# David-OConnor/molchanica

Hardware: AMD Instinct MI355X
Metric: MD atom-updates/sec (and steps/sec), 1M-atom solvated box (higher is better)
Workload: dtype f32

## Files before the change

molchanica_amd/csrc/mdx_nonbonded_impl.h:

```cpp
#pragma once
#include "mdx_internal.h"
#include "mdx_bonded_dev.h"
#include "mdx_pair_dev.h"
#include <algorithm>
#include <cfloat>
#include <cstdlib>
#include <type_traits>

constexpr int NB_WAVES = MDX_NB_WAVES;
#ifdef NB_DRAIN_TRACE
extern uint4* g_mdx_drain; extern size_t g_mdx_drain_cap; extern uint32_t g_mdx_drain_n; extern int g_mdx_drain_on;
#endif
#ifndef NB_ASM_PAIR
#define NB_ASM_PAIR 0
#endif
#ifndef NB_HALF_FLUSH
#define NB_HALF_FLUSH 0
#endif

template <bool BIAS, bool R2OUT>
__device__ __forceinline__ void pair_eval_asm(float xi, float yi, float zi, float qi, float sgi, float epi, const float4 pj,
                                              const float2 lj, float rc2, float bias, float& fx, float& fy, float& fz,
                                              float& g0, float& g1, float& g2, float& r2_out) {
    float dx, dy, dz, r2, t1, t2, t3, t4;
    if (BIAS) {
        asm volatile(
            "v_sub_f32 %[dy], %[yi], %[yj]\n\t"
            "v_sub_f32 %[dx], %[xi], %[xj]\n\t"
            "v_fma_f32 %[r2], %[dy], %[dy], %[bias]\n\t"
            "v_sub_f32 %[dz], %[zi], %[zj]\n\t"
            "v_fmac_f32 %[r2], %[dx], %[dx]\n\t"
            "v_fmac_f32 %[r2], %[dz], %[dz]\n\t"
            : [dx] "=&v"(dx), [dy] "=&v"(dy), [dz] "=&v"(dz), [r2] "=&v"(r2)
            : [xi] "v"(xi), [yi] "v"(yi), [zi] "v"(zi), [xj] "v"(pj.x), [yj] "v"(pj.y), [zj] "v"(pj.z), [bias] "v"(bias));
    } else {
        asm volatile(
            "v_sub_f32 %[dy], %[yi], %[yj]\n\t"
            "v_sub_f32 %[dx], %[xi], %[xj]\n\t"
            "v_mul_f32 %[r2], %[dy], %[dy]\n\t"
            "v_sub_f32 %[dz], %[zi], %[zj]\n\t"
            "v_fmac_f32 %[r2], %[dx], %[dx]\n\t"
            "v_fmac_f32 %[r2], %[dz], %[dz]\n\t"
            : [dx] "=&v"(dx), [dy] "=&v"(dy), [dz] "=&v"(dz), [r2] "=&v"(r2)
            : [xi] "v"(xi), [yi] "v"(yi), [zi] "v"(zi), [xj] "v"(pj.x), [yj] "v"(pj.y), [zj] "v"(pj.z));
    }
    if (R2OUT) r2_out = r2;
    asm volatile(
        "v_cmpx_gt_f32 vcc, %[rc2], %[r2]\n\t"
        "v_rsq_f32 %[r2], %[r2]\n\t"
        "v_add_f32 %[t1], %[sgi], %[ljx]\n\t"
        "v_mul_f32 %[t1], %[t1], %[t1]\n\t"
        "v_mul_f32 %[t2], %[epi], %[ljy]\n\t"
        "v_mul_f32 %[t3], %[r2], %[r2]\n\t"
        "v_mul_f32 %[t1], %[t1], %[t3]\n\t"
        "v_mul_f32 %[t4], %[t1], %[t1]\n\t"
        "v_mul_f32 %[t1], %[t1], %[t4]\n\t"
        "v_mul_f32 %[t2], %[t2], %[t1]\n\t"
        "v_fma_f32 %[t1], %[t1], 2.0, -1.0\n\t"
        "v_mul_f32 %[t1], %[t2], %[t1]\n\t"
        "v_mul_f32 %[t2], %[qi], %[qj]\n\t"
        "v_fmac_f32 %[t1], %[t2], %[r2]\n\t"
        "v_mul_f32 %[t1], %[t3], %[t1]\n\t"
        "v_fmac_f32 %[fx], %[dx], %[t1]\n\t"
        "v_fmac_f32 %[fy], %[dy], %[t1]\n\t"
        "v_fmac_f32 %[fz], %[dz], %[t1]\n\t"
        "v_fma_f32 %[g0], -%[dx], %[t1], %[g0]\n\t"
        "v_fma_f32 %[g1], -%[dy], %[t1], %[g1]\n\t"
        "v_fma_f32 %[g2], -%[dz], %[t1], %[g2]\n\t"
        "s_mov_b64 exec, -1\n\t"
        : [fx] "+v"(fx), [fy] "+v"(fy), [fz] "+v"(fz), [g0] "+v"(g0), [g1] "+v"(g1), [g2] "+v"(g2), [r2] "+v"(r2),
          [t1] "=&v"(t1), [t2] "=&v"(t2), [t3] "=&v"(t3), [t4] "=&v"(t4)
        : [rc2] "s"(rc2), [sgi] "v"(sgi), [epi] "v"(epi), [ljx] "v"(lj.x), [ljy] "v"(lj.y), [qi] "v"(qi), [qj] "v"(pj.w),
          [dx] "v"(dx), [dy] "v"(dy), [dz] "v"(dz)
        : "vcc");
}

template <bool ENERGY, int COUL, bool GEOM, bool SAMECUT, bool MASKED>
__device__ __forceinline__ void chunk_pairs(const float4* __restrict__ sx, const float2* __restrict__ sl,
                                            unsigned long long mask, float xi, float yi, float zi, float qi,
                                            float sgi, float epi, const NbParams& p, float& fx, float& fy,
                                            float& fz, double& elj, double& ecoul, double& evir) {
    float e1 = 0.f, e2 = 0.f, e3 = 0.f;
#pragma unroll 8
    for (int jj = 0; jj < 64; ++jj) {
        const bool allowed = MASKED ? (bool)((mask >> jj) & 1ull) : true;
        pair_eval<ENERGY, COUL, GEOM, SAMECUT, false>(xi, yi, zi, qi, sgi, epi, sx[jj], sl[jj], allowed, p, fx, fy, fz,
                                               e1, e2, nullptr, ENERGY ? &e3 : nullptr);
    }
    if (ENERGY) { elj += (double)e1; ecoul += (double)e2; evir += (double)e3; }
}

template <bool ENERGY, int COUL, bool GEOM, bool SAMECUT>
__global__ __launch_bounds__(NB_WAVES * 64) void nb_tile_kernel(NbArgs a) {
    if (a.gate && *a.gate > a.thr_bits) return;
    __shared__ float4 s_xyzq[NB_WAVES][64];
    __shared__ float2 s_lj[NB_WAVES][64];
    const int lane = threadIdx.x & 63, wave = threadIdx.x >> 6;
    const uint32_t nblocks = (a.T + NB_WAVES - 1) / NB_WAVES;
    const uint32_t per_xcd = (nblocks + 7) >> 3;
    const uint32_t blk = (blockIdx.x & 7u) * per_xcd + (blockIdx.x >> 3);
    if (blk >= nblocks) return;
    const uint32_t t = blk * NB_WAVES + wave;
    if (t >= a.T) return;

    const uint32_t islot = t * MDX_TILE + lane;
    const float4 pi = a.posq[islot];
    const float2 li = a.lj[islot];
    const ListCounts cnt = a.counts[t];
    const uint32_t e0 = a.entry_off[t];
    const uint32_t nmc = cnt.n_masked >> 3, nchunks = (cnt.n_masked + cnt.n_plain) >> 3;
    const uint32_t mbase = a.mchunk_off[t];
    float4* sx = s_xyzq[wave];
    float2* sl = s_lj[wave];

    float fx = 0.f, fy = 0.f, fz = 0.f;
    double elj = 0.0, ecoul = 0.0, evir = 0.0;

    float4 nj = make_float4(0.f, 0.f, 0.f, 0.f);
    float2 nl = make_float2(0.f, 0.f);
    uint32_t ncode = 13;
    if (nchunks) {
        const uint2 ent = a.entries[e0 + (lane >> 3)];
        const uint32_t js = ent.x * MDX_CLUSTER + (lane & 7);
        nj = a.posq[js]; nl = a.lj[js]; ncode = ent.y & 31u;
    }
    for (uint32_t c = 0; c < nchunks; ++c) {
        {
            const int kx = (int)(ncode % 3u) - 1, ky = (int)((ncode / 3u) % 3u) - 1, kz = (int)(ncode / 9u) - 1;
            nj.x += (float)kx * a.p.shift[0];
            nj.y += (float)ky * a.p.shift[1];
            nj.z += (float)kz * a.p.shift[2];
            sx[lane] = nj;
            sl[lane] = nl;
        }
        WAVE_LDS_SYNC();
        if (c + 1 < nchunks) {
            const uint2 ent = a.entries[e0 + (c + 1) * 8 + (lane >> 3)];
            const uint32_t js = ent.x * MDX_CLUSTER + (lane & 7);
            nj = a.posq[js]; nl = a.lj[js]; ncode = ent.y & 31u;
        }
        if (c < nmc) {
            const unsigned long long m = a.masks[(size_t)(mbase + c) * 64 + lane];
            chunk_pairs<ENERGY, COUL, GEOM, SAMECUT, true>(sx, sl, m, pi.x, pi.y, pi.z, pi.w, li.x, li.y, a.p,
                                                           fx, fy, fz, elj, ecoul, evir);
        } else {
            chunk_pairs<ENERGY, COUL, GEOM, SAMECUT, false>(sx, sl, ~0ull, pi.x, pi.y, pi.z, pi.w, li.x, li.y,
                                                            a.p, fx, fy, fz, elj, ecoul, evir);
        }
        WAVE_LDS_SYNC();
    }
    a.force[islot] = make_float4(fx, fy, fz, 0.f);
    if (ENERGY) {
        if (!(a.slot_flags[islot] & 2u)) { elj = 0.0; ecoul = 0.0; evir = 0.0; }
#pragma unroll
        for (int m = 32; m > 0; m >>= 1) {
            elj += __shfl_xor(elj, m);
            ecoul += __shfl_xor(ecoul, m);
            evir += __shfl_xor(evir, m);
        }
        if (lane == 0) {
            double* q = a.energy + EN_COUNT + 8 + MDX_ESTRIDE * (blk & (MDX_EPART - 1));
            atomicAdd(q, 0.5 * elj); atomicAdd(q + 1, 0.5 * ecoul); atomicAdd(q + 2, 0.5 * evir);
        }
    }
}


template <bool ENERGY, int COUL, bool GEOM, bool SAMECUT, int WPT, bool HALF, bool ALCH, int DUAL, int BW, bool STEP = false, bool UNI = false>
__device__ __forceinline__ void nb_cluster_body(const NbArgs& a, const bool owned_prune, float4 (*s_xyzq)[64], float4 (*s_lj)[64],
                                                float (*s_red)[3][64], float (*s_ownj)[64], float4 (*s_g)[64],
                                                unsigned long long (*s_mask)[64], const float4* __restrict__ etab = nullptr) {
    const int lane = threadIdx.x & 63, wave = __builtin_amdgcn_readfirstlane(threadIdx.x >> 6);
    constexpr int SPLIT = BW < WPT ? WPT / BW : 1;
    static_assert(!UNI || (!ENERGY && !GEOM && !ALCH && !STEP), "the constant-sigma^2 body: force-only, Lorentz-Berthelot, no alchemical window");
    static_assert(SPLIT == 1 || HALF, "a tile split over workgroups returns its i-forces through atomics");
    constexpr int TPB = SPLIT > 1 ? 1 : BW / WPT;
    const uint32_t ntiles = a.tile_order ? a.t_count : a.T;
    const uint32_t nblocks = SPLIT > 1 ? ntiles * SPLIT : (ntiles + TPB - 1) / TPB;
    const uint32_t per_xcd = (nblocks + 7) >> 3;
    constexpr bool TAIL = WPT == 1 && HALF && DUAL != 0 && !STEP && BW == 1;
    const bool tail_on = TAIL && a.tail_w > 1u;
    const uint32_t blk = (a.xcd_interleave || tail_on) ? blockIdx.x : (blockIdx.x & 7u) * per_xcd + (blockIdx.x >> 3);
    if (!tail_on && blk >= nblocks) return;
    const int tib = SPLIT > 1 ? 0 : wave / WPT;
// ... 68 lines not shown
                if (a.st_prune_out && !(pw <= a.st_path_thr)) *a.st_prune_out = 1u;
                if (any_viol) { *a.st_viol = 1u; if (a.st_disp_out) atomicMax(a.st_disp_out, __float_as_uint(1.0e20f)); }
            }
            if (WPT == 1 && a.b_role_off) {
                const uint32_t rb = a.b_role_off[s], re = a.b_role_off[s + 1];
                if (re > rb) {
                    float bx = 0.f, by = 0.f, bz = 0.f;
                    RoleEnergies en;
                    for (uint32_t k = rb; k < re; ++k) role_eval_step<false>(a.b_roles[k], a.b_prm, x, a.posq, a.st_fprev, a.b_p, bx, by, bz, en);
                    float* const fb_ = reinterpret_cast<float*>(a.force) + (size_t)s * 4;
                    unsafeAtomicAdd(fb_, bx); unsafeAtomicAdd(fb_ + 1, by); unsafeAtomicAdd(fb_ + 2, bz);
                }
            }
        }
        s_xyzq[wave][lane] = x;
        WAVE_LDS_SYNC();
#pragma unroll
        for (int ci = 0; ci < 8; ++ci) {
            const float4 pi = s_xyzq[wave][ci * MDX_CLUSTER + ii];
            const float2 li = a.lj[t * MDX_TILE + ci * MDX_CLUSTER + ii];
            xi[ci] = pi.x; yi[ci] = pi.y; zi[ci] = pi.z; qi[ci] = pi.w; sgi[ci] = li.x; epi[ci] = li.y;
            fx[ci] = 0.f; fy[ci] = 0.f; fz[ci] = 0.f;
        }
        WAVE_LDS_SYNC();
    } else {
#pragma unroll
    for (int ci = 0; ci < 8; ++ci) {
        const uint32_t s = t * MDX_TILE + ci * MDX_CLUSTER + ii;
        const float4 pi = a.posq[s];
        const float2 li = UNI ? make_float2(0.f, reinterpret_cast<const float*>(a.lj)[2 * s + 1]) : a.lj[s];
        xi[ci] = pi.x; yi[ci] = pi.y; zi[ci] = pi.z; qi[ci] = pi.w; sgi[ci] = li.x; epi[ci] = li.y;
        fx[ci] = 0.f; fy[ci] = 0.f; fz[ci] = 0.f;
    }
    }
    ListCounts cnt = a.counts[t_ok ? t : 0];
    if (!t_ok) { cnt.n_masked = 0; cnt.n_plain = 0; }
    const uint32_t e0 = a.entry_off[t_ok ? t : 0];
    const uint2* __restrict__ const entries = DUAL == 1 ? a.entries_in : a.entries;
    const uint32_t nmc = cnt.n_masked >> 3;
    const uint32_t nchunks = DUAL == 1 ? (t_ok ? a.inner_nch[t * 8 + part] : 0u) : (cnt.n_masked + cnt.n_plain) >> 3;
    const uint32_t mbase = a.mchunk_off[t_ok ? t : 0];
    float4* sx = s_xyzq[wave];
    float4* const sl = s_lj[wave];
    const float* __restrict__ const lj_eps = reinterpret_cast<const float*>(a.lj) + 1;
    double elj = 0.0, ecoul = 0.0, evir = 0.0, ecross = 0.0, edudl = 0.0;
    uint32_t own_bits = 0xFFu;
    if (ENERGY && !a.energy_all) {
        own_bits = 0;
#pragma unroll
        for (int ci = 0; ci < 8; ++ci)
            own_bits |= ((a.slot_flags[t * MDX_TILE + ci * MDX_CLUSTER + ii] >> 1) & 1u) << ci;
    }

    float4 nj = make_float4(0.f, 0.f, 0.f, 0.f), nf = nj;
    float2 nl = make_float2(0.f, 0.f);
    uint32_t ny = 13, njc = 0;
    float nown = 0.f;
    unsigned long long nmq = ~0ull;
    uint2 ent_n = make_uint2(0u, 13u);
    if ((uint32_t)part < nchunks) {
        const uint2 ent = entries[e0 + part * 8 + (lane >> 3)];
        if ((uint32_t)part < nmc) nmq = a.masks[(size_t)(mbase + part) * 64 + lane];
        if ((uint32_t)part + wv < nchunks) ent_n = entries[e0 + (part + wv) * 8 + (lane >> 3)];
        const uint32_t js = ent.x * MDX_CLUSTER + (lane & 7);
        nj = a.posq[js]; ny = ent.y; njc = ent.x;
        if (UNI) nl.y = lj_eps[2 * js]; else nl = a.lj[js];
        if (STEP) nf = a.st_fprev[js];
        if (ENERGY && HALF) nown = a.energy_all ? 1.0f : (float)((a.slot_flags[js] >> 1) & 1u);
    }
    float* const fbase = reinterpret_cast<float*>(a.force);
    const bool jsel_x = ii == 0 || ii == 7, jsel_y = ii == 1 || ii == 6;
    const uint32_t jlane_off = (uint32_t)(jj * 4 + ii) * 4u;
    float4* const sg = s_g[HALF ? wave : 0];
    constexpr bool prune = DUAL == 2;
    uint32_t kept = 0;
#ifdef NB_HALF_STATS
    uint32_t dbg_jh = 0, dbg_ih = 0, dbg_q = 0, dbg_pairs = 0;
#endif
    const uint32_t c_first = nmc + (TAIL ? (((uint32_t)part + wv - (nmc & (wv - 1u))) & (wv - 1u)) : ((uint32_t)part + WPT - nmc % WPT) % WPT);
    uint32_t wcur = 0;
    if (HALF && NB_HALF_FLUSH) __builtin_amdgcn_s_waitcnt(0x0F70);
    const float rc2_s = __builtin_bit_cast(float, __builtin_amdgcn_readfirstlane(__builtin_bit_cast(int, a.p.rc2_lj)));
    auto chunk_pass = [&](auto masked_tag, const uint32_t c_begin, const uint32_t c_end) __attribute__((always_inline)) {
    constexpr bool MASKED_CHUNK = decltype(masked_tag)::value;
    for (uint32_t c = c_begin; c < c_end; c += wv) {
        const uint32_t cur_y = ny, cur_jc = njc;
        constexpr bool masked = MASKED_CHUNK;
        if (masked) s_mask[wave][lane] = nmq;
        if (ENERGY && HALF) s_ownj[wave][lane] = nown;
        if (HALF && NB_HALF_FLUSH) {
            const bool live = ((ny >> 8) & 0xFFu) != 0u;
            sg[lane] = make_float4(0.f, 0.f, 0.f, __uint_as_float(live ? njc * MDX_CLUSTER + (uint32_t)ii : t * MDX_TILE + lane));
        }
        {
            const uint32_t code = ny & 31u;
            const int kx = (int)(code % 3u) - 1, ky = (int)((code / 3u) % 3u) - 1, kz = (int)(code / 9u) - 1;
            if (STEP) nj = step_pos(nj, nf);
            nj.x += (float)kx * a.p.shift[0];
            nj.y += (float)ky * a.p.shift[1];
            nj.z += (float)kz * a.p.shift[2];
            sx[lane] = nj;
            if (UNI) sl[lane].x = nl.y; else *reinterpret_cast<float2*>(&sl[lane]) = nl;
        }
        WAVE_LDS_SYNC();
        if (c + wv < nmc) nmq = a.masks[(size_t)(mbase + c + wv) * 64 + lane];
        if (c + wv < nchunks) {
            const uint32_t js = ent_n.x * MDX_CLUSTER + (lane & 7);
            nj = a.posq[js]; ny = ent_n.y; njc = ent_n.x;
            if (UNI) nl.y = lj_eps[2 * js]; else nl = a.lj[js];
            if (STEP) nf = a.st_fprev[js];
            if (ENERGY && HALF) nown = a.energy_all ? 1.0f : (float)((a.slot_flags[js] >> 1) & 1u);
            if (c + 2 * wv < nchunks) ent_n = entries[e0 + (c + 2 * wv) * 8 + (lane >> 3)];
        }
        float celj = 0.f, cecoul = 0.f, cevir = 0.f, cecross = 0.f, cedudl = 0.f;
        uint32_t newy = cur_y & 0xFFu;
#pragma unroll 1
        for (int e = 0; e < 8; ++e) {
            const float4 pj = sx[e * 8 + jj];
            const float2 lj = UNI ? make_float2(0.f, sl[e * 8 + jj].x) : *reinterpret_cast<const float2*>(&sl[e * 8 + jj]);
            const uint32_t im = (__builtin_amdgcn_readlane(cur_y, e * 8) >> 8) & 0xFFu;
            if (im == 0) continue;
            uint32_t newm = 0;
            const int x8 = MASKED_CHUNK ? (int)(~(uint32_t)reinterpret_cast<const uint8_t*>(&s_mask[wave][lane])[e]) : 0;
            float g[3] = {-0.f, -0.f, -0.f};
            float wj = 0.f;
            if (ENERGY && HALF) wj = 0.5f * s_ownj[wave][e * 8 + jj];
#pragma unroll
            for (int ci = 0; ci < 8; ++ci) {
                if (im & (1u << ci)) {
                    float e1 = 0.f, e2 = 0.f, e3 = 0.f, e4 = 0.f, e5 = 0.f;
                    const float bias = MASKED_CHUNK ? __int_as_float((x8 << (31 - ci)) >> 31) : 0.f;
                    float r2v = 0.f;
                    constexpr bool ASM_PAIR = NB_ASM_PAIR && !ENERGY && COUL == CM_SHIFTED && !GEOM && SAMECUT && HALF && !ALCH && !UNI;
                    if constexpr (ASM_PAIR)
                        pair_eval_asm<MASKED_CHUNK, prune>(xi[ci], yi[ci], zi[ci], qi[ci], sgi[ci], epi[ci], pj, lj, rc2_s, bias, fx[ci], fy[ci], fz[ci],
                                                           g[0], g[1], g[2], r2v);
                    else
                    pair_eval<ENERGY, COUL, GEOM, SAMECUT, true, HALF, ALCH, MASKED_CHUNK, UNI>(xi[ci], yi[ci], zi[ci], qi[ci], sgi[ci], epi[ci],
                                                                             pj, lj, true, a.p, fx[ci], fy[ci],
                                                                             fz[ci], e1, e2, g, ENERGY ? &e3 : nullptr,
                                                                             (ENERGY && ALCH) ? &e4 : nullptr, bias,
                                                                             prune ? &r2v : nullptr, (ENERGY && ALCH) ? &e5 : nullptr, etab);
                    if (prune) {
                        const unsigned long long bb = __ballot(r2v < a.rin2);
                        if (bb != 0ull) newm |= 1u << ci;
#ifdef NB_HALF_STATS
                        if (bb != 0ull) {
                            const unsigned long long ilo = 0x0F0F0F0F0F0F0F0Full;
                            dbg_jh += ((uint32_t)bb != 0u) + ((bb >> 32) != 0ull);
                            dbg_ih += ((bb & ilo) != 0ull) + ((bb & ~ilo) != 0ull);
                            dbg_q += (((uint32_t)bb & 0x0F0F0F0Fu) != 0u) + (((uint32_t)bb & 0xF0F0F0F0u) != 0u) +
                                     (((uint32_t)(bb >> 32) & 0x0F0F0F0Fu) != 0u) + (((uint32_t)(bb >> 32) & 0xF0F0F0F0u) != 0u);
                            dbg_pairs += __popcll(bb);
                        }
#endif
                    }
                    if (ENERGY && HALF) {
                        const float w = wj + (((own_bits >> ci) & 1u) ? 0.5f : 0.f);
                        celj += w * e1; cecoul += w * e2; cevir += w * e3; cecross += w * e4; cedudl += w * e5;
                    } else if (ENERGY && ((own_bits >> ci) & 1u)) { celj += e1; cecoul += e2; cevir += e3; cecross += e4; cedudl += e5; }
                }
            }
            if (prune) {
                kept += __popc(newm);
                if (jj == e) newy |= newm << 8;
            }
            if (HALF && NB_HALF_FLUSH) {
#pragma unroll
                for (int d = 0; d < 3; ++d) {
                    g[d] = dpp_xadd<0xB1>(g[d]);
                    g[d] = dpp_xadd<0x4E>(g[d]);
                    g[d] = dpp_xadd<0x141>(g[d]);
                }
                if (ii < 3) reinterpret_cast<float*>(sg)[(e * 8 + jj) * 4 + ii] = ii == 0 ? g[0] : (ii == 1 ? g[1] : g[2]);
            } else if (HALF) {
                const float v = jforce_reduce8(g, jsel_x, jsel_y);
                typedef __attribute__((address_space(1))) char gchar;
                gchar* frow = (gchar*)(fbase + (size_t)__builtin_amdgcn_readlane(cur_jc, e * 8) * (MDX_CLUSTER * 4));
                asm("" : "+s"(frow));
                if (ii < 3) {
                    uint32_t off = jlane_off;
                    asm("" : "+v"(off));
#ifdef NB_EXP_NOATOMIC
                    if (v == 1.2345e30f)
#endif
                    unsafeAtomicAdd((float*)(frow + off), v);
                }
            }
        }
        if (ENERGY) { elj += (double)celj; ecoul += (double)cecoul; evir += (double)cevir; ecross += (double)cecross; edudl += (double)cedudl; }
        if (prune) {
            if (masked) {
                if (ii == 0) a.entries_in[e0 + c * 8 + jj] = make_uint2(cur_jc, newy);
            } else {
                const bool alive = ii == 0 && (newy >> 8) != 0u;
                const unsigned long long bal = __ballot(alive);
                if (alive) {
                    const uint32_t k = wcur + (uint32_t)__popcll(bal & ((1ull << lane) - 1ull));
                    a.entries_in[e0 + (c_first + (k >> 3) * wv) * 8 + (k & 7u)] = make_uint2(cur_jc, newy);
                }
                wcur += (uint32_t)__popcll(bal);
            }
        }
        WAVE_LDS_SYNC();
        if (HALF && NB_HALF_FLUSH) {
            __builtin_amdgcn_s_waitcnt(0x0F70);
            const float* const sgf = reinterpret_cast<const float*>(sg);
#pragma unroll
            for (int k = 0; k < 3; ++k) {
                const uint32_t fidx = (uint32_t)(k * 64 + lane), atom = (fidx * 171u) >> 9, comp = fidx - 3u * atom;
                const uint32_t slot = __float_as_uint(sgf[atom * 4 + 3]);
                unsafeAtomicAdd(fbase + (size_t)slot * 4 + comp, sgf[atom * 4 + comp]);
            }
        }
    }
    };
#ifndef NB_SPLIT_MASKED
#define NB_SPLIT_MASKED 1
#endif
    if (NB_SPLIT_MASKED) {
        const uint32_t c_mid = c_first < nchunks ? c_first : nchunks;
        chunk_pass(std::true_type{}, (uint32_t)part, c_mid);
        chunk_pass(std::false_type{}, c_mid, nchunks);
    } else chunk_pass(std::true_type{}, (uint32_t)part, nchunks);
    float ox = 0.f, oy = 0.f, oz = 0.f;
#pragma unroll
    for (int ci = 0; ci < 8; ++ci) {
        float x = fx[ci], y = fy[ci], z = fz[ci];
#pragma unroll
        for (int m = 8; m < 64; m <<= 1) {
            x += __shfl_xor(x, m); y += __shfl_xor(y, m); z += __shfl_xor(z, m);
        }
        if (jj == ci) { ox = x; oy = y; oz = z; }
    }
    float* const fi = fbase + (size_t)(t * MDX_TILE + lane) * 4;
    constexpr bool IFORCE_ROWS = HALF && NB_IFORCE_ROWS && !STEP;
    if (prune && t_ok) {
        const uint32_t nfull = (wcur + 7u) >> 3;
        if ((uint32_t)lane < nfull * 8u - wcur) {
            const uint32_t k = wcur + (uint32_t)lane;
            a.entries_in[e0 + (c_first + (k >> 3) * wv) * 8 + (k & 7u)] = make_uint2(a.T * MDX_CL_PER_TILE, 13u);
        }
        if (lane == 0) a.inner_nch[t * 8 + part] = nfull ? c_first + (nfull - 1u) * wv + 1u : nmc;
    }
    if (prune) {
        if (!STEP && part == 0 && t_ok && (owned_prune || !(a.slot_flags[t * MDX_TILE + lane] & 2u))) {
            const uint32_t s = t * MDX_TILE + lane;
            if (a.path) {
                const float4 x = a.posq[s], r = a.ref[s];
                const float dx = x.x - r.x, dy = x.y - r.y, dz = x.z - r.z;
                a.path[s] = 0.f; a.dprune[s] = __builtin_sqrtf(dx * dx + dy * dy + dz * dz);
            } else a.ref[s].w = 0.f;
        }
        if (lane == 0 && kept) atomicAdd(a.inner_count + ((blk * BW + wave) & (MDX_EPART - 1)), (unsigned long long)kept);
        if (lane == 0 && blk == 0 && wave == 0) atomicAdd(a.inner_count + MDX_EPART, 1ull);
#ifdef NB_HALF_STATS
        if (lane == 0) {
            atomicAdd(a.inner_count + MDX_EPART + 1, (unsigned long long)dbg_jh); atomicAdd(a.inner_count + MDX_EPART + 2, (unsigned long long)dbg_ih);
            atomicAdd(a.inner_count + MDX_EPART + 3, (unsigned long long)dbg_q); atomicAdd(a.inner_count + MDX_EPART + 4, (unsigned long long)kept);
            atomicAdd(a.inner_count + MDX_EPART + 5, (unsigned long long)dbg_pairs);
        }
#endif
    }
    if (WPT > 1) {
        s_red[wave][0][lane] = ox; s_red[wave][1][lane] = oy; s_red[wave][2][lane] = oz;
        __syncthreads();
        if ((SPLIT > 1 ? wave == 0 : part == 0) && t_ok) {
            const int w0 = SPLIT > 1 ? 0 : tib * WPT;
            ox = s_red[w0][0][lane]; oy = s_red[w0][1][lane]; oz = s_red[w0][2][lane];
#pragma unroll
            for (int w = 1; w < (SPLIT > 1 ? BW : WPT); ++w) { ox += s_red[w0 + w][0][lane]; oy += s_red[w0 + w][1][lane]; oz += s_red[w0 + w][2][lane]; }
            if (IFORCE_ROWS) iforce_add_rows(fbase + (size_t)t * (MDX_TILE * 4), sx, lane, ox, oy, oz);
            else if (HALF) { unsafeAtomicAdd(fi, ox); unsafeAtomicAdd(fi + 1, oy); unsafeAtomicAdd(fi + 2, oz); }
            else a.force[t * MDX_TILE + lane] = make_float4(ox, oy, oz, 0.f);
        }
    } else {
// ... 75 lines not shown
        }
        bonded_workgroup<STEP>(a, blockIdx.x - a.pair_grid, BW * 64);
        return;
    }
    __shared__ float4 s_xyzq[BW][64];
    __shared__ float4 s_lj[BW][64];
    __shared__ float s_red[WPT > 1 ? BW : 1][3][64];
    __shared__ float s_ownj[(ENERGY && HALF) ? BW : 1][64];
    __shared__ float4 s_g[HALF ? BW : 1][64];
    __shared__ unsigned long long s_mask[BW][64];
    extern __shared__ float4 s_dyn_etab[];
    const float4* etab = nullptr;
    if (COUL == CM_EWALD_TAB && !ENERGY && !ALCH) {
        for (uint32_t k = threadIdx.x; k < a.p.etab_n; k += BW * 64) s_dyn_etab[k] = a.p.etab[k];
        __syncthreads();
        etab = reinterpret_cast<const float4*>(reinterpret_cast<const char*>(s_dyn_etab) - ((EWALD_TAB_CBITS >> a.p.etab_shift) << 4));
    }
#ifdef NB_DRAIN_TRACE
    const unsigned long long drain_t0 = wall_clock64();
#endif
    if (DUAL == 0) {
        nb_cluster_body<ENERGY, COUL, GEOM, SAMECUT, WPT, HALF, ALCH, 0, BW, false, UNI>(a, true, s_xyzq, s_lj, s_red, s_ownj, s_g, s_mask, etab);
    } else {
        const bool owned_prune = (a.force_prune | *a.prune_flag) != 0u;
        const bool want_prune = owned_prune || (a.prune_flag2 && *a.prune_flag2 != 0u);
        if (DUAL >= 3) {
#if NB_MERGED_NOINLINE
            static_assert(!UNI, "the experiment has the general bodies only");
            if (want_prune) nb_cluster_body_call<ENERGY, COUL, GEOM, SAMECUT, WPT, HALF, ALCH, 2, BW>(a, owned_prune, s_xyzq, s_lj, s_red, s_ownj, s_g, s_mask, etab);
            else nb_cluster_body_call<ENERGY, COUL, GEOM, SAMECUT, WPT, HALF, ALCH, 1, BW>(a, owned_prune, s_xyzq, s_lj, s_red, s_ownj, s_g, s_mask, etab);
#else
            if (want_prune) nb_cluster_body<ENERGY, COUL, GEOM, SAMECUT, WPT, HALF, ALCH, 2, BW, STEP, UNI>(a, owned_prune, s_xyzq, s_lj, s_red, s_ownj, s_g, s_mask, etab);
            else nb_cluster_body<ENERGY, COUL, GEOM, SAMECUT, WPT, HALF, ALCH, 1, BW, STEP, UNI>(a, owned_prune, s_xyzq, s_lj, s_red, s_ownj, s_g, s_mask, etab);
#endif
        } else {
            if (want_prune != (DUAL == 2)) return;
            nb_cluster_body<ENERGY, COUL, GEOM, SAMECUT, WPT, HALF, ALCH, DUAL == 2 ? 2 : 1, BW, false, UNI>(a, owned_prune, s_xyzq, s_lj, s_red, s_ownj, s_g, s_mask, etab);
        }
#ifdef NB_DRAIN_TRACE
        if (DUAL == 3 && a.drain) {
            __builtin_amdgcn_s_waitcnt(0);
            const unsigned long long t1 = wall_clock64();
            if ((threadIdx.x & 63u) == 0u) {
                uint4* const o = a.drain + 2 * ((size_t)blockIdx.x * BW + (threadIdx.x >> 6));
                o[0] = make_uint4((uint32_t)drain_t0, (uint32_t)(drain_t0 >> 32), (uint32_t)t1, (uint32_t)(t1 >> 32));
                o[1] = make_uint4(__builtin_amdgcn_s_getreg(4 | (31 << 11)), __builtin_amdgcn_s_getreg(20 | (31 << 11)), want_prune ? 1u : 0u, 1u);
            }
        }
#endif
    }
}

template <bool ENERGY, int COUL, bool G, bool S, int WPT, bool HALF, int DUAL>
static bool launch_cluster(bool uni, dim3 g, dim3 b, uint32_t lds, hipStream_t st, const NbArgs& a) {
    if constexpr (!ENERGY && !G && COUL != CM_SOFT) {
        if (uni) {
            hipLaunchKernelGGL((nb_cluster_kernel<false, COUL, false, S, WPT, HALF, false, DUAL, false, 1, true>), g, b, lds, st, a);
            return true;
        }
    }
    hipLaunchKernelGGL((nb_cluster_kernel<ENERGY, COUL, G, S, WPT, HALF, false, DUAL>), g, b, lds, st, a);
    return false;
}

template <bool ENERGY, int COUL>
void launch_variant(mdx_handle* h, const NbArgs& a_in, bool geom, bool samecut) {
    NbArgs a = a_in;
    const bool uni = h->uni_lj && !h->alch_on && !geom && a.p.uni_c != 0.f;
    bool uni_used = false;
    const int var = mdx_nb_variant(h);
    int wpt = 1;
    const bool half = var == 5;
    if (var == 2) wpt = (a.T < mdx_wpt8_below(h)) ? 8 : 4;
    if (half) wpt = mdx_nb_wpt_half(h, a.T);
    if (var == 4) wpt = 4;
    const uint32_t bw = std::max(wpt, NB_WAVES);
    const uint32_t tpb = (var == 1) ? NB_WAVES : bw / wpt;
    const uint32_t nblocks = ((a.tile_order ? a.t_count : a.T) + tpb - 1) / tpb;
    const uint32_t grid = ((nblocks + 7) / 8) * 8;
    if (nblocks == 0) return;
    dim3 g(grid), b(bw * 64);
    if (half && wpt == 1 && a.inner && !ENERGY && !a.st_fprev && h->tail_w > 1u && h->tile_lpt_on && a.tile_order == h->d.tile_lpt && !a.xcd_interleave) {
        a.tail_group = (a.T + 7u) >> 3;
        const uint32_t tail = std::min(h->tail_tiles, a.tail_group);
        a.tail_w = h->tail_w; a.tail_head = a.tail_group - tail;
        g = dim3(8u * (a.tail_head + a.tail_w * tail));
    }
    if (a.inner) {
        uint32_t n_tail = 0;
        for (uint32_t x = 0; a.tail_w && x < 8u; ++x) {
            const uint32_t in_range = a.T > x * a.tail_group ? std::min(a.T - x * a.tail_group, a.tail_group) : 0u;
            n_tail += in_range > a.tail_head ? in_range - a.tail_head : 0u;
        }
        h->pair_info_tail[0] = a.tail_w; h->pair_info_tail[1] = n_tail;
    }
#ifdef NB_DRAIN_TRACE
    if (a.inner && g_mdx_drain_on) {
        const size_t want = (size_t)g.x * bw * 2;
        if (want > g_mdx_drain_cap) {
            if (g_mdx_drain) (void)hipFree(g_mdx_drain);
            (void)hipMalloc((void**)&g_mdx_drain, sizeof(uint4) * want);
            g_mdx_drain_cap = want;
        }
        (void)hipMemsetAsync(g_mdx_drain, 0, sizeof(uint4) * want, h->stream);
        a.drain = g_mdx_drain; g_mdx_drain_n = (uint32_t)(g.x * bw);
    }
#endif
    static const uint32_t lds_pad_env = [] { const char* e = std::getenv("MDX_NB_LDS_PAD"); return e ? (uint32_t)std::atoi(e) : 0u; }();
    const uint32_t lds_pad = ((h->pme_on && h->pme_overlap && !ENERGY) ? lds_pad_env : 0u) +
                             ((COUL == CM_EWALD_TAB && !ENERGY) ? a.p.etab_n * (uint32_t)sizeof(float4) : 0u);
    static const bool dual_merged = [] { const char* e = std::getenv("MDX_DUAL_MERGED"); return !(e && e[0] == '0'); }();
    static const bool merge_all = [] { const char* e = std::getenv("MDX_DUAL_MERGED"); return !(e && (e[0] == '0' || e[0] == '1')); }();
    static const int split_env = [] { const char* e = std::getenv("MDX_TILE_SPLIT"); return e ? (e[0] == '0' ? 0 : 1) : -1; }();
    const bool split2 = split_env >= 0 ? split_env == 1 : (a.tile_order ? a.t_count : a.T) < 1024u;
    static const bool fb_all = [] { const char* e = std::getenv("MDX_FUSE_BONDED"); return e && e[0] == '2'; }();
    auto note = [&](int dual, int w, int split, int fb) {
        uint32_t* const o = a.inner ? h->pair_info_step : h->pair_info_any;
        o[0] = (uint32_t)w; o[1] = (uint32_t)dual; o[2] = half ? 1u : 0u; o[3] = (uint32_t)COUL; o[4] = ENERGY ? 1u : 0u;
        o[5] = (uint32_t)split; o[6] = (uint32_t)fb; o[7] = a.tile_order ? a.t_count : a.T;
    };
#define NB_STEP(G, S)                                                                                                 \
    do {                                                                                                               \
// ... 19 lines not shown
#define NB_DUAL(G, S, D)                                                                                              \
    do {                                                                                                               \
        if (ENERGY) break;                                                                                             \
        if (fb_all && a.b_S && (wpt == 2 || wpt == 4)) {     \
            NbArgs af = a; af.pair_grid = grid;                                                                        \
            const dim3 gf(grid + (uint32_t)(((size_t)a.b_S * 4 + bw * 64 - 1) / (bw * 64)));                           \
            if (wpt == 2) hipLaunchKernelGGL((nb_cluster_kernel<false, COUL, G, S, 2, true, false, D, true>), gf, b, lds_pad, h->stream, af); \
            else hipLaunchKernelGGL((nb_cluster_kernel<false, COUL, G, S, 4, true, false, D, true>), gf, b, lds_pad, h->stream, af);          \
            h->bonded_fused = true; note(D, wpt, 1, 1);                                                                \
            break;                                                                                                     \
        }                                                                                                              \
        note(D, wpt == 8 || wpt == 2 || wpt == 1 ? wpt : 4, 1, 0);                                                     \
        if (wpt == 8) hipLaunchKernelGGL((nb_cluster_kernel<false, COUL, G, S, 8, true, false, D>), g, b, lds_pad, h->stream, a); \
        else if (wpt == 2) hipLaunchKernelGGL((nb_cluster_kernel<false, COUL, G, S, 2, true, false, D>), g, b, lds_pad, h->stream, a); \
        else if (wpt == 1) uni_used = launch_cluster<false, COUL, G, S, 1, true, D>(uni, g, b, lds_pad, h->stream, a);                 \
        else hipLaunchKernelGGL((nb_cluster_kernel<false, COUL, G, S, 4, true, false, D>), g, b, lds_pad, h->stream, a);               \
    } while (0)
#define NB_LAUNCH(G, S)                                                                                    \
    do {                                                                                                   \
        note(0, var == 1 ? 0 : ((h->alch_on && wpt != 8) ? 4 : wpt), 1, 0);    \
        if (h->alch_on && wpt == 8) hipLaunchKernelGGL((nb_cluster_kernel<ENERGY, COUL, G, S, 8, true, COUL != CM_EWALD_TAB>), g, b, lds_pad, h->stream, a); \
        else if (h->alch_on) hipLaunchKernelGGL((nb_cluster_kernel<ENERGY, COUL, G, S, 4, true, COUL != CM_EWALD_TAB>), g, b, lds_pad, h->stream, a); \
        else if (a.st_fprev) { NB_STEP(G, S); }                                                                    \
        else if (var == 1) hipLaunchKernelGGL((nb_tile_kernel<ENERGY, COUL, G, S>), g, b, lds_pad, h->stream, a);     \
        else if (half && a.inner && dual_merged && wpt == 8 && split2 && !ENERGY) {    \
            NbArgs af = a;                                                                                         \
            const uint32_t nb2 = (a.tile_order ? a.t_count : a.T) * 2u;                                            \
            af.pair_grid = ((nb2 + 7) / 8) * 8;                                                                    \
            const dim3 gf(af.pair_grid + (a.b_S ? (uint32_t)(((size_t)a.b_S * 4 + 255) / 256) : 0u)), bf(256);     \
            if (a.b_S) { hipLaunchKernelGGL((nb_cluster_kernel<false, COUL, G, S, 8, true, false, 4, false, 2>), gf, bf, lds_pad, h->stream, af); h->bonded_fused = true; note(4, 8, 2, 0); } \
            else { hipLaunchKernelGGL((nb_cluster_kernel<false, COUL, G, S, 8, true, false, 3, false, 2>), gf, bf, lds_pad, h->stream, af); note(3, 8, 2, 0); } \
        }                                                                                                          \
        else if (half && a.inner && dual_merged && wpt == 8 && a.b_S && !ENERGY) {                                 \
            NbArgs af = a; af.pair_grid = grid;                                                                    \
            const dim3 gf(grid + (uint32_t)(((size_t)a.b_S * 4 + bw * 64 - 1) / (bw * 64)));                       \
            hipLaunchKernelGGL((nb_cluster_kernel<false, COUL, G, S, 8, true, false, 4>), gf, b, lds_pad, h->stream, af); \
            h->bonded_fused = true; note(4, 8, 1, 0);                                                              \
        }                                                                                                          \
        else if (half && a.inner && dual_merged && (wpt == 8 || merge_all)) { NB_DUAL(G, S, 3); }                  \
        else if (half && a.inner) { if (!a.force_prune) NB_DUAL(G, S, 1); NB_DUAL(G, S, 2); }    \
        else if (half && wpt == 8) hipLaunchKernelGGL((nb_cluster_kernel<ENERGY, COUL, G, S, 8, true>), g, b, lds_pad, h->stream, a); \
        else if (half && wpt == 2) hipLaunchKernelGGL((nb_cluster_kernel<ENERGY, COUL, G, S, 2, true>), g, b, lds_pad, h->stream, a); \
        else if (half && wpt == 1) uni_used = launch_cluster<ENERGY, COUL, G, S, 1, true, 0>(uni, g, b, lds_pad, h->stream, a);    \
        else if (half) hipLaunchKernelGGL((nb_cluster_kernel<ENERGY, COUL, G, S, 4, true>), g, b, lds_pad, h->stream, a); \
        else if (wpt == 8) uni_used = launch_cluster<ENERGY, COUL, G, S, 8, false, 0>(uni, g, b, lds_pad, h->stream, a);           \
        else if (wpt == 4) uni_used = launch_cluster<ENERGY, COUL, G, S, 4, false, 0>(uni, g, b, lds_pad, h->stream, a);           \
        else hipLaunchKernelGGL((nb_cluster_kernel<ENERGY, COUL, G, S, 1, false>), g, b, lds_pad, h->stream, a);        \
    } while (0)
    if (geom) { if (samecut) NB_LAUNCH(true, true); else NB_LAUNCH(true, false); }
    else      { if (samecut) NB_LAUNCH(false, true); else NB_LAUNCH(false, false); }
#undef NB_LAUNCH
#undef NB_DUAL
#undef NB_STEP
    if (a.inner || (h->nb_step >= 0 && a.gate)) h->pair_body_step = uni_used ? 1u : 0u;
    h->pair_body_any = uni_used ? 1u : 0u;
}
```

molchanica_amd/csrc/mdx_pair_dev.h:

```cpp
#pragma once
#include "mdx_internal.h"

struct NbParams;
void mdx_fill_nb_params(const mdx_handle* h, NbParams& p, int* mode_out, bool* geom_out, bool* samecut_out);

#define WAVE_LDS_SYNC()                                        \
    do {                                                       \
        __builtin_amdgcn_fence(__ATOMIC_SEQ_CST, "workgroup"); \
        __builtin_amdgcn_wave_barrier();                       \
    } while (0)

template <int CTRL>
__device__ __forceinline__ float dpp_xadd(float v) {
    return v + __int_as_float(__builtin_amdgcn_update_dpp(0, __float_as_int(v), CTRL, 0xF, 0xF, true));
}

__device__ __forceinline__ float jforce_reduce8(const float g[3], const bool sel_x, const bool sel_y) {
    float q[3];
#pragma unroll
    for (int d = 0; d < 3; ++d) q[d] = dpp_xadd<0x4E>(dpp_xadd<0xB1>(g[d]));
    float v = dpp_xadd<0x141>(sel_x ? q[0] : (sel_y ? q[1] : q[2]));
    asm volatile("" : "+v"(v));
    return v;
}

#ifndef NB_IFORCE_ROWS
#define NB_IFORCE_ROWS 1
#endif

__device__ __forceinline__ void iforce_add_rows(float* __restrict__ rows, float4* strip, const int lane, const float ox, const float oy, const float oz) {
    strip[lane] = make_float4(ox, oy, oz, 0.f);
    WAVE_LDS_SYNC();
    const float* const w = reinterpret_cast<const float*>(strip);
#pragma unroll
    for (int k = 0; k < 4; ++k) {
        const float v = w[k * 64 + lane];
        if ((lane & 3) != 3) unsafeAtomicAdd(rows + k * 64 + lane, v);
    }
}

struct NbArgs {
    uint32_t T;
    const float4* posq; const float2* lj;
    const ListCounts* counts; const uint32_t* entry_off; const uint32_t* mchunk_off;
    const uint2* entries; const unsigned long long* masks;
    float4* force; double* energy;
    const uint8_t* slot_flags;
    NbParams p;
    const uint32_t* gate; uint32_t thr_bits;
    uint32_t inner;
    uint32_t force_prune;
    const uint32_t* prune_flag;
    float rin2;
    uint2* entries_in;
    uint32_t* inner_nch;
    float4* ref; unsigned long long* inner_count;
    float* path; float* dprune;
    uint32_t xcd_interleave;
    const uint32_t* tile_order; uint32_t t_first, t_count;
    const uint32_t* prune_flag2;
    uint32_t energy_all;
    uint32_t pair_grid, b_S;
    const uint32_t* b_role_off; const RoleRec* b_roles; const float4* b_prm;
    BondedParams b_p;
    const float4* st_fprev; float4* st_yout; float4* st_fnext; float4* st_vel;
    float st_dt, st_path_thr;
    uint32_t st_last;
    float st_grant;
    float st_kick;
    uint32_t* st_disp_out;
    uint32_t* st_prune_out;
    uint32_t* st_viol;
    uint32_t tail_w, tail_head, tail_group;
#ifdef NB_DRAIN_TRACE
    uint4* drain;
#endif
// ... 100 lines not shown
```

molchanica_amd/md_state.py:

```python
from __future__ import annotations

import ctypes as C
import os

import numpy as np

from ._abi import (CCommDiag, CFlexOpts, CHBond, CConfig, CEnergies, CRefineOpts, CSearchOpts, CStats, CSystem, FLEX_DIHEDRALS, FORCE,
                   MDX_EDEVICE, MDX_ENAN, MDX_EOOM, MDX_EPARAM, MDX_OK, POS, POSE_MAX_ATOMS, POSE_MAX_TORSIONS, VEL, MdConfig, MdSystem)

_HERE = os.path.dirname(os.path.abspath(__file__))
LIB_PATH = os.environ.get("MDX_LIB") or os.path.join(_HERE, "libmdx.so")


class ParamError(ValueError):
    """The reference's `ParamError { descrip }` (src/md/mod.rs:967)."""


class DeviceError(RuntimeError):
    """HIP/device failure (MDX_EDEVICE / MDX_EOOM); the reference degrades to its CPU path here
    (src/util.rs:1072-1119) — this library has none and says so loudly."""


class BlowUpError(FloatingPointError):
    """Non-finite state (MDX_ENAN); cf. the stop criteria at sol_shrinking_box.rs:776-789."""
# ... 553 lines not shown

    _n_waters = 0
    _water_first = 0
    _water_sites = 0

    def set_water_layout(self, first_atom: int, n_waters: int, sites_per_water: int):
        _check(load_library().mdx_set_water_layout(self._h, int(first_atom), int(n_waters), int(sites_per_water)))
        self._water_first, self._n_waters, self._water_sites = int(first_atom), int(n_waters), int(sites_per_water)

    def water(self, which: str = "posit") -> dict:
        n = self._n_waters
        arr = {k: np.empty((n, 3), dtype=np.float32) for k in (("o", "h0", "h1", "m") if self._water_sites == 4 else ("o", "h0", "h1"))}
        _check(load_library().mdx_water_download(self._h, POS if which == "posit" else FORCE, arr["o"].ctypes.data_as(_fp),
                                                 arr["h0"].ctypes.data_as(_fp), arr["h1"].ctypes.data_as(_fp),
                                                 arr["m"].ctypes.data_as(_fp) if "m" in arr else None))
        return arr

    def set_hbond_detection(self, is_heavy_nosf, max_h_acc_dist: float = 2.5, min_angle_deg: float = 120.0):
        if is_heavy_nosf is None:
            _check(load_library().mdx_set_hbond_detection(self._h, None, 0.0, 0.0))
            return
        m = np.ascontiguousarray(is_heavy_nosf, dtype=np.uint8).reshape(self.n_atoms)
        _check(load_library().mdx_set_hbond_detection(self._h, m.ctypes.data, float(max_h_acc_dist), float(min_angle_deg)))

    def flush_snapshot_queues(self):
        _check(load_library().mdx_flush_snapshot_queues(self._h))

    @property
    def time_ps(self) -> float:
        return float(load_library().mdx_time_ps(self._h))

    def profile(self, enable=True):
        _check(load_library().mdx_profile(self._h, int(enable)))

    def stats(self) -> dict:
        s = CStats()
        _check(load_library().mdx_get_stats(self._h, C.byref(s)))
        return s.as_dict()

    def pair_launch_info(self) -> dict:
        out = (C.c_uint32 * 24)()
        _check(load_library().mdx_pair_launch_info(self._h, out))
        keys = ("waves_per_tile", "dual", "half", "coulomb", "energy", "workgroups_per_tile", "bonded_workgroups", "tiles")
        return {"step": dict(zip(keys, (int(v) for v in out[0:8]))), "any": dict(zip(keys, (int(v) for v in out[8:16]))),
                "inner_lists_from_rebuilds": int(out[16]), "last_rebuild_wrote_the_inner_list": bool(out[17]),
                "water_step_launches": int(out[18]), "water_step_mixed_launches": int(out[19]),
                "one_launch_steps": int(out[20]), "kicks_beyond_grant": int(out[21]),
                "tail": {"waves_per_tile": int(out[22]), "tiles": int(out[23])}}

    def pair_body_info(self) -> dict:
        out = (C.c_uint32 * 4)()
        _check(load_library().mdx_pair_body_info(self._h, out))
        return {"eligible": bool(out[0]), "step": bool(out[1]), "any": bool(out[2]), "c_bits": int(out[3]),
                "c": float(np.array([out[3]], np.uint32).view(np.float32)[0])}

    def skin(self):
        v, t = C.c_float(), C.c_int()
        _check(load_library().mdx_get_skin(self._h, C.byref(v), C.byref(t)))
        return float(v.value), bool(t.value)

    def computation_time(self) -> float:
        return float(self.stats()["wall_ms_sum"])

    def comm_init(self, unique_id: bytes, rank: int, world: int):
        assert len(unique_id) == 128
        _check(load_library().mdx_comm_init(self._h, bytes(unique_id), int(rank), int(world)))

    def comm_init_fabric(self, fabric: "Fabric", rank: int):
        self._fabric = fabric
        _check(load_library().mdx_comm_init_fabric(self._h, fabric.ptr, int(rank)))

    def comm_init_shm(self, name: str, rank: int, world: int):
        _check(load_library().mdx_comm_init_shm(self._h, name.encode(), int(rank), int(world)))

    def comm_init_null(self, rank: int, world: int):
        _check(load_library().mdx_comm_init_null(self._h, int(rank), int(world)))

    def comm_selftest(self):
        _check(load_library().mdx_comm_selftest(self._h))

    def comm_selftest_fault(self):
        _check(load_library().mdx_comm_selftest_fault(self._h))

    def comm_debug_partition(self, n_atoms: int) -> dict:
        cls = np.zeros(n_atoms, np.uint8); owner = np.zeros(n_atoms, np.uint8); code = np.zeros(n_atoms, np.uint8)
        mask = np.zeros(n_atoms, np.uint32)
        ns, nr = C.c_uint32(), C.c_uint32()
        lib = load_library()
        _check(lib.mdx_comm_debug_partition(self._h, cls.ctypes.data, owner.ctypes.data, code.ctypes.data, mask.ctypes.data,
                                            C.byref(ns), C.byref(nr), None, None, 0))
        sid = np.zeros(max(ns.value, 1), np.uint32); rid = np.zeros(max(nr.value, 1), np.uint32)
        _check(lib.mdx_comm_debug_partition(self._h, None, None, None, None, C.byref(ns), C.byref(nr), sid.ctypes.data, rid.ctypes.data,
                                            max(ns.value, nr.value, 1)))
        return dict(cls=cls, owner=owner, image_code=code, send_mask=mask, send_ids=sid[:ns.value], recv_ids=rid[:nr.value])

    def pme_info(self) -> dict:
        on, a, b, c = C.c_int(), C.c_uint64(), C.c_uint64(), C.c_uint64()
        _check(load_library().mdx_pme_info(self._h, C.byref(on), C.byref(a), C.byref(b), C.byref(c)))
        return dict(slab_on=bool(on.value), mesh_bytes_sent=a.value, transpose_bytes_sent=b.value, replicated_mesh_bytes=c.value)

    def pme_brick_overflows(self) -> int:
        n = C.c_uint64()
        _check(load_library().mdx_pme_brick_overflows(self._h, C.byref(n)))
        return int(n.value)

    def set_hydrogen_constraint(self, kind: str, order: int = 4, iters: int = 1, shake_tolerance: float = 0.0) -> str:
# ... 118 lines not shown
```

Baseline: 2.236 billion.

## Double-buffer j-cluster prefetch across two register sets in plain nonbonded chunks

For the half-list, uniform-LJ, single-wave-per-tile, non-energy, non-step kernel variant, the plain (unmasked) chunk loop now alternates between two register sets of prefetched j-cluster data. Each set loads its next chunk two strides ahead, so global loads get more time to land before they are needed. The image-shift computation is factored into a helper, and the launch reports whether the two-set path was used. The cost is extra VGPR pressure, which may lower occupancy, and more code complexity.

```diff
diff --git a/molchanica_amd/csrc/mdx_nonbonded_impl.h b/molchanica_amd/csrc/mdx_nonbonded_impl.h
--- a/molchanica_amd/csrc/mdx_nonbonded_impl.h
+++ b/molchanica_amd/csrc/mdx_nonbonded_impl.h
@@ -16,6 +16,12 @@
 #endif
 #ifndef NB_HALF_FLUSH
 #define NB_HALF_FLUSH 0
+#endif
+#ifndef NB_SPLIT_MASKED
+#define NB_SPLIT_MASKED 1
+#endif
+#ifndef NB_LATCH2
+#define NB_LATCH2 1
 #endif
 
 template <bool BIAS, bool R2OUT>
@@ -75,6 +81,10 @@
         : "vcc");
 }
 
+constexpr bool nb_latch2(bool half, bool uni, int wpt, bool energy, bool alch, bool step) {
+    return NB_LATCH2 && NB_SPLIT_MASKED && half && !NB_HALF_FLUSH && uni && wpt == 1 && !energy && !alch && !step;
+}
+
 template <bool ENERGY, int COUL, bool GEOM, bool SAMECUT, bool MASKED>
 __device__ __forceinline__ void chunk_pairs(const float4* __restrict__ sx, const float2* __restrict__ sl,
                                             unsigned long long mask, float xi, float yi, float zi, float qi,
@@ -126,10 +136,9 @@
     }
     for (uint32_t c = 0; c < nchunks; ++c) {
         {
-            const int kx = (int)(ncode % 3u) - 1, ky = (int)((ncode / 3u) % 3u) - 1, kz = (int)(ncode / 9u) - 1;
-            nj.x += (float)kx * a.p.shift[0];
-            nj.y += (float)ky * a.p.shift[1];
-            nj.z += (float)kz * a.p.shift[2];
+            float rx, ry, rz;
+            image_shift_row(ncode, a.p.shift, rx, ry, rz);
+            nj.x += rx; nj.y += ry; nj.z += rz;
             sx[lane] = nj;
             sl[lane] = nl;
         }
@@ -304,22 +313,30 @@
             own_bits |= ((a.slot_flags[t * MDX_TILE + ci * MDX_CLUSTER + ii] >> 1) & 1u) << ci;
     }
 
-    float4 nj = make_float4(0.f, 0.f, 0.f, 0.f), nf = nj;
-    float2 nl = make_float2(0.f, 0.f);
-    uint32_t ny = 13, njc = 0;
-    float nown = 0.f;
-    unsigned long long nmq = ~0ull;
-    uint2 ent_n = make_uint2(0u, 13u);
-    if ((uint32_t)part < nchunks) {
-        const uint2 ent = entries[e0 + part * 8 + (lane >> 3)];
-        if ((uint32_t)part < nmc) nmq = a.masks[(size_t)(mbase + part) * 64 + lane];
-        if ((uint32_t)part + wv < nchunks) ent_n = entries[e0 + (part + wv) * 8 + (lane >> 3)];
-        const uint32_t js = ent.x * MDX_CLUSTER + (lane & 7);
-        nj = a.posq[js]; ny = ent.y; njc = ent.x;
-        if (UNI) nl.y = lj_eps[2 * js]; else nl = a.lj[js];
-        if (STEP) nf = a.st_fprev[js];
-        if (ENERGY && HALF) nown = a.energy_all ? 1.0f : (float)((a.slot_flags[js] >> 1) & 1u);
-    }
+    struct JSet {
+        float4 nj, nf;
+        float2 nl;
+        uint32_t ny, njc;
+        float nown;
+        unsigned long long nmq;
+        uint2 ent;
+    };
+    constexpr bool LATCH2 = nb_latch2(HALF, UNI, WPT, ENERGY, ALCH, STEP);
+    JSet S0 = {make_float4(0.f, 0.f, 0.f, 0.f), make_float4(0.f, 0.f, 0.f, 0.f), make_float2(0.f, 0.f), 13u, 0u, 0.f, ~0ull, make_uint2(0u, 13u)};
+    JSet S1 = S0;
+    auto prime = [&](JSet& X, const uint32_t c0) __attribute__((always_inline)) {
+        if (c0 < nchunks) {
+            const uint2 ent = entries[e0 + c0 * 8 + (lane >> 3)];
+            if (c0 < nmc) X.nmq = a.masks[(size_t)(mbase + c0) * 64 + lane];
+            if (c0 + wv < nchunks) X.ent = entries[e0 + (c0 + wv) * 8 + (lane >> 3)];
+            const uint32_t js = ent.x * MDX_CLUSTER + (lane & 7);
+            X.nj = a.posq[js]; X.ny = ent.y; X.njc = ent.x;
+            if (UNI) X.nl.y = lj_eps[2 * js]; else X.nl = a.lj[js];
+            if (STEP) X.nf = a.st_fprev[js];
+            if (ENERGY && HALF) X.nown = a.energy_all ? 1.0f : (float)((a.slot_flags[js] >> 1) & 1u);
+        }
+    };
+    prime(S0, (uint32_t)part);
     float* const fbase = reinterpret_cast<float*>(a.force);
     const bool jsel_x = ii == 0 || ii == 7, jsel_y = ii == 1 || ii == 6;
     const uint32_t jlane_off = (uint32_t)(jj * 4 + ii) * 4u;
@@ -333,36 +350,48 @@
     uint32_t wcur = 0;
     if (HALF && NB_HALF_FLUSH) __builtin_amdgcn_s_waitcnt(0x0F70);
     const float rc2_s = __builtin_bit_cast(float, __builtin_amdgcn_readfirstlane(__builtin_bit_cast(int, a.p.rc2_lj)));
-    auto chunk_pass = [&](auto masked_tag, const uint32_t c_begin, const uint32_t c_end) __attribute__((always_inline)) {
-    constexpr bool MASKED_CHUNK = decltype(masked_tag)::value;
-    for (uint32_t c = c_begin; c < c_end; c += wv) {
-        const uint32_t cur_y = ny, cur_jc = njc;
+    auto chunk = [&](auto masked_tag, auto two_tag, const uint32_t c, JSet& X) __attribute__((always_inline)) {
+        constexpr bool MASKED_CHUNK = decltype(masked_tag)::value, TWO = decltype(two_tag)::value;
+        const uint32_t ps = TWO ? 2u * wv : wv;
+        uint32_t cur_y = X.ny, cur_jc = X.njc;
+        if (TWO) asm volatile("" : "+v"(cur_y), "+v"(cur_jc));
         constexpr bool masked = MASKED_CHUNK;
-        if (masked) s_mask[wave][lane] = nmq;
-        if (ENERGY && HALF) s_ownj[wave][lane] = nown;
+        if (masked) s_mask[wave][lane] = X.nmq;
+        if (ENERGY && HALF) s_ownj[wave][lane] = X.nown;
         if (HALF && NB_HALF_FLUSH) {
-            const bool live = ((ny >> 8) & 0xFFu) != 0u;
-            sg[lane] = make_float4(0.f, 0.f, 0.f, __uint_as_float(live ? njc * MDX_CLUSTER + (uint32_t)ii : t * MDX_TILE + lane));
+            const bool live = ((X.ny >> 8) & 0xFFu) != 0u;
+            sg[lane] = make_float4(0.f, 0.f, 0.f, __uint_as_float(live ? X.njc * MDX_CLUSTER + (uint32_t)ii : t * MDX_TILE + lane));
         }
         {
-            const uint32_t code = ny & 31u;
-            const int kx = (int)(code % 3u) - 1, ky = (int)((code / 3u) % 3u) - 1, kz = (int)(code / 9u) - 1;
-            if (STEP) nj = step_pos(nj, nf);
-            nj.x += (float)kx * a.p.shift[0];
-            nj.y += (float)ky * a.p.shift[1];
-            nj.z += (float)kz * a.p.shift[2];
-            sx[lane] = nj;
-            if (UNI) sl[lane].x = nl.y; else *reinterpret_cast<float2*>(&sl[lane]) = nl;
+            const uint32_t code = X.ny & 31u;
+            if (STEP) X.nj = step_pos(X.nj, X.nf);
+            float rx, ry, rz;
+            image_shift_row(code, a.p.shift, rx, ry, rz);
+            X.nj.x += rx; X.nj.y += ry; X.nj.z += rz;
+            sx[lane] = X.nj;
+            if (UNI) sl[lane].x = X.nl.y; else *reinterpret_cast<float2*>(&sl[lane]) = X.nl;
         }
         WAVE_LDS_SYNC();
-        if (c + wv < nmc) nmq = a.masks[(size_t)(mbase + c + wv) * 64 + lane];
-        if (c + wv < nchunks) {
-            const uint32_t js = ent_n.x * MDX_CLUSTER + (lane & 7);
-            nj = a.posq[js]; ny = ent_n.y; njc = ent_n.x;
-            if (UNI) nl.y = lj_eps[2 * js]; else nl = a.lj[js];
-            if (STEP) nf = a.st_fprev[js];
-            if (ENERGY && HALF) nown = a.energy_all ? 1.0f : (float)((a.slot_flags[js] >> 1) & 1u);
-            if (c + 2 * wv < nchunks) ent_n = entries[e0 + (c + 2 * wv) * 8 + (lane >> 3)];
+        if constexpr (TWO) {
+            const uint32_t ce = c + 2u * ps < nchunks ? c + 2u * ps : c;
+            const uint32_t js = X.ent.x * MDX_CLUSTER + (lane & 7);
+            X.ny = X.ent.y; X.njc = X.ent.x;
+            asm volatile("" : "+v"(X.ny), "+v"(X.njc));
+            X.nj = a.posq[js];
+            X.nl.y = lj_eps[2 * js];
+            X.ent = entries[e0 + ce * 8 + (lane >> 3)];
+        } else {
+        if (c + ps < nmc) X.nmq = a.masks[(size_t)(mbase + c + ps) * 64 + lane];
+        if (c + ps < nchunks) {
+            const uint32_t js = X.ent.x * MDX_CLUSTER + (lane & 7);
+            X.ny = X.ent.y; X.njc = X.ent.x;
+            if (!STEP) asm volatile("" : "+v"(X.ny), "+v"(X.njc));
+            X.nj = a.posq[js];
+            if (UNI) X.nl.y = lj_eps[2 * js]; else X.nl = a.lj[js];
+            if (STEP) X.nf = a.st_fprev[js];
+            if (ENERGY && HALF) X.nown = a.energy_all ? 1.0f : (float)((a.slot_flags[js] >> 1) & 1u);
+            if (c + 2 * ps < nchunks) X.ent = entries[e0 + (c + 2 * ps) * 8 + (lane >> 3)];
+        }
         }
         float celj = 0.f, cecoul = 0.f, cevir = 0.f, cecross = 0.f, cedudl = 0.f;
         uint32_t newy = cur_y & 0xFFu;
@@ -465,7 +494,27 @@
                 unsafeAtomicAdd(fbase + (size_t)slot * 4 + comp, sgf[atom * 4 + comp]);
             }
         }
-    }
+    };
+    auto chunk_pass = [&](auto masked_tag, const uint32_t c_begin, const uint32_t c_end) __attribute__((always_inline)) {
+        for (uint32_t c = c_begin; c < c_end; c += wv) chunk(masked_tag, std::false_type{}, c, S0);
+    };
+    auto plain_pass2 = [&](const uint32_t c_begin, const uint32_t c_end) __attribute__((always_inline)) {
+        if (c_begin >= c_end) return;
+        {
+            const uint32_t js = S0.ent.x * MDX_CLUSTER + (lane & 7);
+            S1.ny = S0.ent.y; S1.njc = S0.ent.x;
+            S1.nj = a.posq[js];
+            S1.nl.y = lj_eps[2 * js];
+            const uint32_t c2 = c_begin + 2u * wv < nchunks ? c_begin + 2u * wv : c_begin, c3 = c_begin + 3u * wv < nchunks ? c_begin + 3u * wv : c_begin;
+            S1.ent = entries[e0 + c3 * 8 + (lane >> 3)];
+            S0.ent = entries[e0 + c2 * 8 + (lane >> 3)];
+        }
+        for (uint32_t c = c_begin; c < c_end; c += wv) {
+            chunk(std::false_type{}, std::true_type{}, c, S0);
+            c += wv;
+            if (c >= c_end) break;
+            chunk(std::false_type{}, std::true_type{}, c, S1);
+        }
     };
 #ifndef NB_SPLIT_MASKED
 #define NB_SPLIT_MASKED 1
@@ -473,7 +522,8 @@
     if (NB_SPLIT_MASKED) {
         const uint32_t c_mid = c_first < nchunks ? c_first : nchunks;
         chunk_pass(std::true_type{}, (uint32_t)part, c_mid);
-        chunk_pass(std::false_type{}, c_mid, nchunks);
+        if constexpr (LATCH2) plain_pass2(c_mid, nchunks);
+        else chunk_pass(std::false_type{}, c_mid, nchunks);
     } else chunk_pass(std::true_type{}, (uint32_t)part, nchunks);
     float ox = 0.f, oy = 0.f, oz = 0.f;
 #pragma unroll
@@ -655,22 +705,22 @@
 }
 
 template <bool ENERGY, int COUL, bool G, bool S, int WPT, bool HALF, int DUAL>
-static bool launch_cluster(bool uni, dim3 g, dim3 b, uint32_t lds, hipStream_t st, const NbArgs& a) {
+static uint32_t launch_cluster(bool uni, dim3 g, dim3 b, uint32_t lds, hipStream_t st, const NbArgs& a) {
     if constexpr (!ENERGY && !G && COUL != CM_SOFT) {
         if (uni) {
             hipLaunchKernelGGL((nb_cluster_kernel<false, COUL, false, S, WPT, HALF, false, DUAL, false, 1, true>), g, b, lds, st, a);
-            return true;
+            return 1u | (nb_latch2(HALF, true, WPT, false, false, false) ? 2u : 0u);
         }
     }
     hipLaunchKernelGGL((nb_cluster_kernel<ENERGY, COUL, G, S, WPT, HALF, false, DUAL>), g, b, lds, st, a);
-    return false;
+    return 0u;
 }
 
 template <bool ENERGY, int COUL>
 void launch_variant(mdx_handle* h, const NbArgs& a_in, bool geom, bool samecut) {
     NbArgs a = a_in;
     const bool uni = h->uni_lj && !h->alch_on && !geom && a.p.uni_c != 0.f;
-    bool uni_used = false;
+    uint32_t uni_used = 0u;
     const int var = mdx_nb_variant(h);
     int wpt = 1;
     const bool half = var == 5;
@@ -796,6 +846,6 @@
 #undef NB_LAUNCH
 #undef NB_DUAL
 #undef NB_STEP
-    if (a.inner || (h->nb_step >= 0 && a.gate)) h->pair_body_step = uni_used ? 1u : 0u;
-    h->pair_body_any = uni_used ? 1u : 0u;
-}
+    if (a.inner || (h->nb_step >= 0 && a.gate)) h->pair_body_step = uni_used;
+    h->pair_body_any = uni_used;
+}
diff --git a/molchanica_amd/csrc/mdx_pair_dev.h b/molchanica_amd/csrc/mdx_pair_dev.h
--- a/molchanica_amd/csrc/mdx_pair_dev.h
+++ b/molchanica_amd/csrc/mdx_pair_dev.h
@@ -22,6 +22,13 @@
     float v = dpp_xadd<0x141>(sel_x ? q[0] : (sel_y ? q[1] : q[2]));
     asm volatile("" : "+v"(v));
     return v;
+}
+
+__device__ __forceinline__ void image_shift_row(const uint32_t code, const float (&shift)[3], float& rx, float& ry, float& rz) {
+    const int kx = (int)(code % 3u) - 1, ky = (int)((code / 3u) % 3u) - 1, kz = (int)(code / 9u) - 1;
+    rx = (float)kx * shift[0];
+    ry = (float)ky * shift[1];
+    rz = (float)kz * shift[2];
 }
 
 #ifndef NB_IFORCE_ROWS
diff --git a/molchanica_amd/md_state.py b/molchanica_amd/md_state.py
--- a/molchanica_amd/md_state.py
+++ b/molchanica_amd/md_state.py
@@ -629,6 +629,7 @@
         out = (C.c_uint32 * 4)()
         _check(load_library().mdx_pair_body_info(self._h, out))
         return {"eligible": bool(out[0]), "step": bool(out[1]), "any": bool(out[2]), "c_bits": int(out[3]),
+                "step_two_sets": bool(out[1] & 2), "any_two_sets": bool(out[2] & 2),
                 "c": float(np.array([out[3]], np.uint32).view(np.float32)[0])}
 
     def skin(self):
```

Measured after the change: 2.264 billion (median of 6 runs). 1.01x the previous value.
